# renzibei/flashws

Hardware: AMD Instinct MI355X
Metric: GiB/s masked WS payload unmasked, device-resident frame batch; % HBM roofline (higher is better)
Workload: dtype u8; 1 GPU; C2: device-resident 65536 x 4 KiB masked BIN frames, descriptor-mode unmask of the packed (sorted) batch, one launch (fws_gpu_unmask_sorted); frames_per_gpu=65536, payload_bytes_per_frame=4096, wire_bytes_per_gpu=268959744, rotating_buffers=4, parallelism=batch split x1 (no collective)

## Files before the change

flashws_amd/csrc/fws_abi.hip:

```cpp
#include <stdlib.h>
#include <string.h>

#include "fws_internal.h"

namespace {

template <typename T>
int dev_alloc(T **p, uint64_t count) {
    *p = nullptr;
    if (count == 0) count = 1;
    return fws_hip_status(hipMalloc((void **)p, count * sizeof(T)));
}

template <typename T>
void dev_free(T *&p) {
    if (p) (void)hipFree(p);
    p = nullptr;
}

void free_plan(fws_plan_ws &w) {
    dev_free(w.block_sums);
    dev_free(w.cbase);
    dev_free(w.unit_first);
    dev_free(w.unit_rec);
    dev_free(w.total);
    dev_free(w.status);
    dev_free(w.ticket);
    dev_free(w.mode);
    dev_free(w.tx_seam);
}

}

int fws_ctx_ensure_plan(fws_gpu_ctx *ctx, uint64_t frames, uint64_t units) {
    if (frames <= ctx->cap_frames && units <= ctx->cap_units && ctx->plan.cbase) return 0;
    if (frames < ctx->cap_frames) frames = ctx->cap_frames;
    if (units < ctx->cap_units) units = ctx->cap_units;
    free_plan(ctx->plan);
    int r;
    if ((r = dev_alloc(&ctx->plan.block_sums, frames / 1024 + 2))) return r;
    if ((r = dev_alloc(&ctx->plan.cbase, frames + 2))) return r;
    if ((r = dev_alloc(&ctx->plan.unit_first, units + 2))) return r;
    if ((r = dev_alloc(&ctx->plan.unit_rec, 4 * (units + 2)))) return r;
    if ((r = dev_alloc(&ctx->plan.total, 2))) return r;
    if ((r = dev_alloc(&ctx->plan.status, frames / 8 + 2))) return r;
    if ((r = dev_alloc(&ctx->plan.ticket, 2))) return r;
    if ((r = dev_alloc(&ctx->plan.mode, sizeof(fws_plan_mode) / 8))) return r;
    if ((r = dev_alloc(&ctx->plan.tx_seam, 4 * (2 * frames + 2)))) return r;
    if ((r = fws_hip_status(hipMemset(ctx->plan.status, 0, (frames / 8 + 2) * 8)))) return r;
    if ((r = fws_hip_status(hipMemset(ctx->plan.ticket, 0, 8)))) return r;
    if ((r = fws_hip_status(hipMemset(ctx->plan.mode, 0, sizeof(fws_plan_mode))))) return r;
    ctx->plan.status_cap = frames / 8 + 2;
    ctx->plan.epoch = 0;
    ctx->cap_frames = frames;
    ctx->cap_units = units;
    ctx->plan.unit_cap = units + 1;
    return 0;
}

int fws_ctx_ensure_seam(fws_gpu_ctx *ctx, uint64_t span) {
    const uint64_t words = 2 * (span / 4096 + 2);
    if (words <= ctx->seam_cap) return 0;
    dev_free(ctx->seam);
    ctx->seam_cap = 0;
    if (int r = fws_hip_status(hipMalloc((void **)&ctx->seam, words * 4))) return r;
    ctx->seam_cap = words;
    return 0;
}

int fws_ctx_ensure_msg(fws_gpu_ctx *ctx, uint64_t frames) {
    fws_msg_ws &m = ctx->msg;
    if (!m.cnext) {
        if (int r = dev_alloc(&m.cnext, 1)) return r;
    }
    if (frames <= m.cap && m.descs) return 0;
    if (frames < m.cap) frames = m.cap;
    dev_free(m.descs);
    dev_free(m.ctl_off);
    dev_free(m.agg);
    dev_free(m.pre);
    m.cap = 0;
    int r;
    if ((r = dev_alloc(&m.descs, frames + 1))) return r;
    if ((r = dev_alloc(&m.ctl_off, frames + 1))) return r;
    if ((r = dev_alloc(&m.agg, 8 * (frames / 256 + 2)))) return r;
    if ((r = dev_alloc(&m.pre, 8 * (frames / 256 + 2)))) return r;
    if ((r = fws_hip_status(hipMemset(m.agg, 0, 8 * (frames / 256 + 2) * 8)))) return r;
    if ((r = fws_hip_status(hipMemset(m.pre, 0, 8 * (frames / 256 + 2) * 8)))) return r;
    m.cap = frames;
    m.last_epoch = 0;
    return 0;
}

extern "C" {

__attribute__((visibility("default"))) int fws_internal_decode_counters(fws_gpu_ctx *ctx, uint32_t *out, int n) {
    if (!ctx || !out || n <= 0 || !ctx->dec.counters) return FWS_ERR_INVALID;
    if (n > 64) n = 64;
    return fws_hip_status(hipMemcpy(out, ctx->dec.counters, (size_t)n * 4, hipMemcpyDeviceToHost));
}

__attribute__((visibility("default"))) int fws_internal_plan_mode(fws_gpu_ctx *ctx, uint64_t *out5) {
    if (!ctx || !out5 || !ctx->plan.mode) return FWS_ERR_INVALID;
    return fws_hip_status(hipMemcpy(out5, ctx->plan.mode, 5 * 8, hipMemcpyDeviceToHost));
}

__attribute__((visibility("default"))) int fws_internal_decode_parse(fws_gpu_ctx *ctx, const void *dev_wire,
                                                                     uint64_t len, fws_frame_info *dev_frames,
                                                                     uint32_t cap, fws_decode_result *dev_result,
                                                                     void *stream) {
    if (!ctx || !dev_result || (len && !dev_wire) || (cap && !dev_frames) || ((uintptr_t)dev_wire & 15u))
        return FWS_ERR_INVALID;
    int r;
    if ((r = fws_hip_status(hipSetDevice(ctx->device))) || (r = fws_decode_prepare(ctx, len, cap, false))) return r;
    return fws_launch_decode(ctx, (uint8_t *)const_cast<void *>(dev_wire), len, dev_frames, cap, dev_result, nullptr,
                             (hipStream_t)stream);
}

int fws_gpu_abi_version(void) { return FWS_GPU_ABI_VERSION; }

int fws_gpu_device_count(int *count) {
    if (!count) return FWS_ERR_INVALID;
    *count = 0;
    hipError_t e = hipGetDeviceCount(count);
    if (e == hipErrorNoDevice) { *count = 0; return 0; }
    return fws_hip_status(e);
}

int fws_gpu_ctx_create(int device, fws_gpu_ctx **out) {
    if (!out) return FWS_ERR_INVALID;
    *out = nullptr;
    int n = 0;
    int r = fws_gpu_device_count(&n);
    if (r) return r;
    if (device < 0 || device >= n) return FWS_ERR_NO_DEVICE;
    hipDeviceProp_t prop;
    if ((r = fws_hip_status(hipGetDeviceProperties(&prop, device)))) return r;
// ... 319 lines not shown
```

flashws_amd/csrc/fws_internal.h:

```cpp
#pragma once

#include <hip/hip_runtime.h>
#include <stdint.h>

#include "fws_gpu.h"

static inline int fws_hip_status(hipError_t e) {
    return e == hipSuccess ? 0 : (FWS_ERR_HIP_BASE - (int)e);
}

constexpr uint64_t kSmallMax = 128u << 10;
constexpr uint32_t kSmallFrames = 256;
constexpr int FWS_SMALL_DECLINED = -30;
int fws_resolve_mode();
int fws_launch_decode_small(uint8_t *wire, uint64_t N, fws_frame_info *frames, uint32_t cap,
                            fws_decode_result *res, hipStream_t s);
struct fws_seg_desc {
    uint64_t cont_off;
    uint64_t hs_off;
    uint32_t u;
    uint32_t key;
    uint32_t L;
    uint32_t fcap;
    uint32_t fbase;
// ... 29 lines not shown
static_assert(sizeof(fws_svc_mail) == 128, "one line");
struct alignas(128) fws_svc_dev {
    uint64_t seqn;
    uint32_t quit, ctr, pad[28];
    fws_svc_req req;
};
int fws_launch_rx_service(fws_svc_mail *mail, const fws_svc_mail *poll, fws_svc_dev *dv, uint32_t seq0,
                          uint32_t workers, uint64_t linger_ticks, uint64_t life_ticks, uint32_t trace, hipStream_t s);
int fws_rx_service_trace_read(unsigned long long *out8);
struct fws_rx_service;
fws_rx_service *fws_ctx_rx_service(fws_gpu_ctx *ctx);
void fws_rx_service_destroy(fws_rx_service *v);
int fws_rx_service_run(fws_rx_service *v, uint8_t *base, const fws_seg_desc *descs, const fws_seg_desc *one,
                       uint32_t nseg, fws_frame_info *frames, fws_decode_result *res, uint32_t *flag,
                       uint32_t flag_seq);
int fws_rx_service_post(fws_rx_service *v, uint8_t *base, const fws_seg_desc *descs, uint32_t nseg,
                        fws_frame_info *frames, fws_decode_result *res, uint32_t *flag, uint32_t flag_seq);
int fws_rx_service_wait(fws_rx_service *v, uint32_t *flag, uint32_t flag_seq);
bool fws_rx_service_can_push(const fws_rx_service *v, uint64_t span);
uint32_t fws_rx_service_workers(const fws_rx_service *v);
int fws_rx_service_push(fws_rx_service *v, const uint8_t *src, uint64_t span, uint8_t *out_dev, const fws_seg_desc &d,
                        fws_frame_info *frames, fws_decode_result *res, uint32_t *flag, uint32_t flag_seq);

struct fws_plan_ws {
    uint64_t *block_sums = nullptr;
    uint64_t *cbase = nullptr;
    uint32_t *unit_first = nullptr;
    uint32_t *unit_rec = nullptr;
    uint64_t *total = nullptr;
    uint64_t *status = nullptr;
    uint32_t *ticket = nullptr;
    uint64_t *mode = nullptr;
    uint32_t *tx_seam = nullptr;
    uint64_t status_cap = 0;
    uint32_t epoch = 0;
    uint64_t unit_cap = 0;
};

struct fws_plan_mode {
    uint64_t byte_space;
    uint64_t s0;
    uint64_t first_po;
    uint64_t last_pe;
    uint64_t n_units;
    uint64_t pad[3];
};

struct fws_node_res {
    uint32_t tail;
    uint32_t cnt;
    uint32_t ent;
    uint32_t kind;
};
struct fws_tail_rec {
    uint64_t exit;
    uint32_t id;
    uint32_t w;
    uint32_t wst;
    uint32_t pad;
};

struct fws_st_node {
    uint32_t sid;
    uint16_t nx;
    uint16_t tail;
    uint16_t cnt;
    uint8_t wt;
    uint8_t pad0;
    uint32_t pad1;
};

struct fws_decode_ws {
    uint64_t max_tiles = 0;
    uint64_t max_surv = 0;
    uint32_t *tile_count = nullptr;
    uint32_t *counters = nullptr;
    uint32_t *cnt_base = nullptr;
    uint32_t parity = 0;
// ... 131 lines not shown
```

flashws_amd/csrc/outplan_kernels.hip:

```cpp
#include "fws_device.h"
#include "fws_internal.h"
#include "outplan_common.h"

namespace fwsk {

template <typename Desc, int kF>
__global__ __launch_bounds__(kBlock) void k_out_plan(const Desc *__restrict__ d, uint32_t n, OutPlanArgs a) {
    out_plan_block<Desc, kF>(d, n, a, plan_block_order(a.ticket));
}

}

using namespace fwsk;

int fws_plan_next_epoch(fws_plan_ws &ws, hipStream_t s) {
    if (++ws.epoch > 0xFFFFu) {
        int r = fws_hip_status(hipMemsetAsync(ws.status, 0, ws.status_cap * 8, s));
        if (r) return r;
        ws.epoch = 1;
    }
    return 0;
}

template <typename Desc>
static int launch_out_plan(const Desc *d, uint32_t n, fws_plan_ws &ws, uint64_t out_cap, uint64_t *out_len,
                           hipStream_t s, const uint32_t *deny = nullptr) {
    if (n == 0) return 0;
    const bool small = n <= 16384u;
    const uint32_t nb = small ? (n + 63u) / 64u : (n + kBlock - 1) / kBlock;
    if (nb > ws.status_cap) return FWS_ERR_CAPACITY;
    int r = fws_plan_next_epoch(ws, s);
    if (r) return r;
    OutPlanArgs a{ws.cbase, ws.unit_first, ws.unit_cap, ws.total, out_len, out_cap, deny, ws.status, ws.ticket, ws.epoch};
    if (small)
        hipLaunchKernelGGL((k_out_plan<Desc, 64>), dim3(nb), dim3(kBlock), 0, s, d, n, a);
    else
        hipLaunchKernelGGL((k_out_plan<Desc, kBlock>), dim3(nb), dim3(kBlock), 0, s, d, n, a);
    return fws_hip_status(hipGetLastError());
}

int fws_launch_gather_plan(const fws_frame_desc *d, uint32_t n, fws_plan_ws &ws, hipStream_t s, uint64_t out_cap,
                           const uint32_t *deny) {
    return launch_out_plan(d, n, ws, out_cap, nullptr, s, deny);
}

int fws_launch_tx_plan(const fws_tx_desc *d, uint32_t n, fws_plan_ws &ws, uint64_t out_cap, uint64_t *out_len,
                       hipStream_t s) {
    return launch_out_plan(d, n, ws, out_cap, out_len, s);
}
```

flashws_amd/csrc/plan_common.h:

```cpp
#pragma once
#include "fws_device.h"

namespace fwsk {

constexpr uint64_t kLbValue = (1ull << 45) - 1;
constexpr uint64_t kLbSorted = 1ull << 45;
constexpr uint64_t kLbAgg = 1ull << 46, kLbPrefix = 2ull << 46;

__device__ __forceinline__ uint64_t lb_load(const uint64_t *p) {
    return __hip_atomic_load(p, __ATOMIC_RELAXED, __HIP_MEMORY_SCOPE_AGENT);
}
__device__ __forceinline__ void lb_store(uint64_t *p, uint64_t v) {
    __hip_atomic_store(p, v, __ATOMIC_RELAXED, __HIP_MEMORY_SCOPE_AGENT);
}

__device__ __forceinline__ uint64_t wave_incl_scan64(uint64_t v, int lane) {
#pragma unroll
    for (int o = 1; o < kWave; o <<= 1) {
        const uint64_t t = __shfl_up(v, o, kWave);
        if (lane >= o) v += t;
    }
    return v;
}

__device__ __forceinline__ uint32_t plan_block_order(uint32_t *ticket) {
    __shared__ uint32_t s_blk;
    if (gridDim.x <= 1024u) return blockIdx.x;
    if (threadIdx.x == 0) s_blk = atomicAdd(ticket, 1u);
    __syncthreads();
    const uint32_t blk = s_blk;
    if (blk == gridDim.x - 1 && threadIdx.x == 0) *ticket = 0u;
    return blk;
}

__device__ __forceinline__ uint64_t block_lookback(uint64_t *status, uint32_t blk, uint64_t agg, bool flag,
                                                   uint32_t epoch, bool *all_flag) {
    __shared__ uint32_t s_pstop[kBlock / kWave];
    __shared__ uint64_t s_lsum[kBlock / kWave];
    __shared__ uint32_t s_lbad[kBlock / kWave];
    const int lane = threadIdx.x & (kWave - 1), w = threadIdx.x / kWave;
    const uint64_t tag = (uint64_t)epoch << 48;
    if (threadIdx.x == 0) lb_store(status + blk, tag | (blk == 0 ? kLbPrefix : kLbAgg) | (flag ? kLbSorted : 0) | agg);
    uint64_t excl = 0;
    bool all = flag;
    for (int64_t j = (int64_t)blk - 1; j >= 0; j -= kBlock) {
        const int64_t idx = j - (int64_t)threadIdx.x;
        uint64_t st = tag | kLbPrefix | kLbSorted;
        if (idx >= 0) {
            do {
                st = lb_load(status + idx);
            } while ((st >> 48) != epoch || (st & (3ull << 46)) == 0);
        }
        const uint64_t pm = __ballot((st & (3ull << 46)) == kLbPrefix);
        if (lane == 0) s_pstop[w] = pm ? (uint32_t)(w * kWave + __builtin_ctzll(pm)) : (uint32_t)kBlock;
        __syncthreads();
        uint32_t stop = kBlock;
#pragma unroll
        for (int i = 0; i < kBlock / kWave; ++i) stop = s_pstop[i] < stop ? s_pstop[i] : stop;
        const bool use = threadIdx.x <= stop && idx >= 0;
        uint64_t v = use ? (st & kLbValue) : 0;
        for (int o = 32; o > 0; o >>= 1) v += __shfl_xor(v, o, kWave);
        const uint64_t vb = __ballot(use && !(st & kLbSorted));
        if (lane == 0) {
            s_lsum[w] = v;
            s_lbad[w] = vb != 0;
        }
        __syncthreads();
#pragma unroll
        for (int i = 0; i < kBlock / kWave; ++i) {
            excl += s_lsum[i];
            all = all && !s_lbad[i];
        }
        __syncthreads();
        if (stop < (uint32_t)kBlock) break;
    }
    if (threadIdx.x == 0 && blk != 0)
        lb_store(status + blk, tag | kLbPrefix | (all ? kLbSorted : 0) | ((excl + agg) & kLbValue));
    *all_flag = all;
    return excl;
}

__device__ __forceinline__ uint32_t wave_max(uint32_t v) {
#pragma unroll
    for (int o = 32; o > 0; o >>= 1) {
        const uint32_t t = (uint32_t)__shfl_xor(v, o, kWave);
        v = t > v ? t : v;
    }
    return v;
}

__device__ __forceinline__ uint64_t readlane64(uint64_t v, int k) {
    const uint32_t lo = __builtin_amdgcn_readlane((uint32_t)v, k), hi = __builtin_amdgcn_readlane((uint32_t)(v >> 32), k);
    return ((uint64_t)hi << 32) | lo;
}

constexpr uint32_t kRunInline = 64;

template <typename Get, typename Fn>
__device__ __forceinline__ void wave_for_runs(uint64_t u0, uint32_t len, Get get, Fn fn) {
    if (wave_max(len) <= kRunInline) {
        const auto ctx = get(-1);
        for (uint32_t k = 0; k < len; ++k) fn(ctx, u0 + k);
        return;
    }
    const int lane = threadIdx.x & (kWave - 1);
    for (int L = 0; L < kWave; ++L) {
        const uint32_t n = __builtin_amdgcn_readlane(len, L);
        if (n == 0) continue;
// ... 27 lines not shown
```

flashws_amd/csrc/unmask_kernels.hip:

```cpp
#include "fws_device.h"
#include "fws_internal.h"
#include "plan_common.h"

namespace fwsk {

#ifndef FWS_UNMASK_WT
#define FWS_UNMASK_WT 1
#endif
template <bool kNT, bool kWT = true>
__device__ __forceinline__ void ustore16(uintptr_t a, u32x4 v) {
    if constexpr (kNT && kWT && FWS_UNMASK_WT != 0) gstore16_wt(a, v);
    else gstore16<kNT>(a, v);
}

constexpr int kPlanItems = 1;
constexpr int kPlanTile = kBlock * kPlanItems;

__device__ __forceinline__ uint64_t wave_incl_scan(uint64_t v, int lane) {
#pragma unroll
    for (int o = 1; o < kWave; o <<= 1) {
        uint64_t t = __shfl_up(v, o, kWave);
        if (lane >= o) v += t;
    }
    return v;
// ... 1 lines not shown

__device__ __forceinline__ uint64_t block_excl_scan(uint64_t v, uint64_t *total) {
    __shared__ uint64_t wsum[kBlock / kWave];
    const int lane = threadIdx.x & (kWave - 1), w = threadIdx.x / kWave;
    uint64_t inc = wave_incl_scan(v, lane);
    if (lane == kWave - 1) wsum[w] = inc;
    __syncthreads();
    uint64_t off = 0, tot = 0;
#pragma unroll
    for (int i = 0; i < kBlock / kWave; ++i) {
        uint64_t s = wsum[i];
        off += (i < w) ? s : 0;
        tot += s;
    }
    __syncthreads();
    *total = tot;
    return off + inc - v;
}

__device__ __forceinline__ uint64_t desc_chunks(const uint8_t *base, const fws_frame_desc &d) {
    return chunks_of((uintptr_t)(base + d.payload_off), d.payload_len);
}

struct PlanArgs {
    uint64_t *cbase;
    uint32_t *unit_first;
    u32x4 *unit_rec;
    uint64_t *total;
    uint64_t *status;
    uint32_t *ticket;
    fws_plan_mode *mode;
    uint64_t unit_cap;
    uint32_t epoch;
};

constexpr uint32_t kRecSlow = 1u << 30;

__device__ __forceinline__ uint32_t rec_clip(uint64_t x, uint64_t U0) {
    return x <= U0 ? 0u : (x >= U0 + 4096u ? 4096u : (uint32_t)(x - U0));
}

__device__ __forceinline__ u32x4 unit_record(uint64_t U0, uint64_t E0, uint64_t E1, uint32_t f, uint64_t poA,
                                             uint64_t peA, uint32_t rkA, bool hasB, uint64_t poB, uint64_t peB,
                                             uint32_t rkB, bool hasC, uint64_t poC) {
    if (U0 < E0 || U0 + 4096u > E1 || (hasC && poC < U0 + 4096u)) return u32x4{f, 0u, kRecSlow, 0u};
    const uint32_t a0 = rec_clip(poA, U0), a1 = rec_clip(peA, U0);
    const uint32_t b0 = hasB ? rec_clip(poB, U0) : 0u, b1 = hasB ? rec_clip(peB, U0) : 0u;
    return u32x4{rkA, hasB ? rkB : 0u, a0 | (a1 << 13), b0 | (b1 << 13)};
}


__global__ __launch_bounds__(kBlock) void k_plan(const uint8_t *base, const fws_frame_desc *__restrict__ d,
                                                 uint32_t n, const uint32_t *__restrict__ n_dev, PlanArgs a) {
    __shared__ uint64_t s_wsum[kBlock / kWave];
    __shared__ uint32_t s_wbad[kBlock / kWave];
    if (n_dev && *n_dev < n) n = *n_dev;
    const int lane = threadIdx.x & (kWave - 1), w = threadIdx.x / kWave;
    const uint32_t blk = plan_block_order(a.ticket);
    if (n == 0) {
        if (blk == 0 && threadIdx.x == 0) {
            a.cbase[0] = 0;
            *a.total = 0;
            *a.mode = fws_plan_mode{0, 0, 0, 0, 0, {0, 0, 0}};
        }
        return;
    }
    const uintptr_t b0 = (uintptr_t)base;
    static_assert(kPlanItems == 1, "k_plan: one frame per thread");
    const uint64_t f = uint64_t(blk) * kPlanTile + threadIdx.x;
    const bool has = f < n, hasB = f + 1 < n, hasC = f + 2 < n;
    fws_frame_desc fa{0, 0, 0, 0}, fb{0, 0, 0, 0};
    if (has) fa = d[f];
    if (hasB) fb = d[f + 1];
    const uint64_t poC = hasC ? d[f + 2].payload_off : 0;
    const uint64_t po0 = d[0].payload_off;
    const uint64_t last_pe = d[n - 1].payload_off + d[n - 1].payload_len;
    const uint64_t poA = fa.payload_off, peA = fa.payload_off + fa.payload_len;
    const uint64_t poB = fb.payload_off, peB = fb.payload_off + fb.payload_len;
    const uint64_t s = has ? chunks_of(b0 + poA, fa.payload_len) : 0;
    const bool srt = !hasB || (peA >= poA && peA <= poB);
    const uint64_t inc = wave_incl_scan64(s, lane);
    const uint64_t bad = __ballot(!srt);
    if (lane == kWave - 1) {
        s_wsum[w] = inc;
        s_wbad[w] = bad != 0;
    }
    __syncthreads();
    uint64_t run0 = inc - s, agg = 0;
    bool blk_sorted = true;
#pragma unroll
    for (int i = 0; i < kBlock / kWave; ++i) {
        run0 += i < w ? s_wsum[i] : 0;
        agg += s_wsum[i];
        blk_sorted = blk_sorted && !s_wbad[i];
    }
    bool all_sorted;
    const uint64_t prefix = block_lookback(a.status, blk, agg, blk_sorted, a.epoch, &all_sorted);
    const uint64_t Sa = (b0 + po0) & ~uint64_t(15);
    const uint64_t S = Sa - b0;
    const uint64_t cap = a.unit_cap;
    const uint64_t nus = b0 + last_pe > Sa ? (b0 + last_pe - Sa + 4095u) / 4096u : 0;
    uint64_t run = prefix + run0;
    uint64_t cu = 0, cue = 0, bu = 0, bue = 0;
    if (has) {
        a.cbase[f] = run;
        if (s) {
            cu = (run + kUnitChunks - 1) / kUnitChunks;
            cue = (run + s + kUnitChunks - 1) / kUnitChunks;
        }
        run += s;
        bu = f == 0 ? 0 : (b0 + poA >= Sa ? (b0 + poA - Sa + 4095u) / 4096u : cap);
        bue = !hasB ? nus : (b0 + poB >= Sa ? (b0 + poB - Sa + 4095u) / 4096u : 0);
        if (f == n - 1) {
            a.cbase[n] = run;
            *a.total = run;
            const bool dense = all_sorted && nus + 1 <= cap && (last_pe - S) <= 2u * (run * 16u) + 65536u;
            fws_plan_mode m{dense ? 1ull : 0ull, S, po0, last_pe, nus, {0, 0, 0}};
            *a.mode = m;
        }
    }
    if (cue > cap) cue = cap;
    if (bue > cap) bue = cap;
    if (!all_sorted) bue = bu;
    if (cue < cu) cue = cu;
    if (bue < bu) bue = bu;
    wave_fill_runs(a.unit_first, cu, (uint32_t)(cue - cu), (uint32_t)f, lane);
    struct RecCtx {
        uint64_t poA, peA, poB, peB, poC;
        uint32_t f, rkA, rkB;
        bool hasB, hasC;
    };
    const RecCtx mine{poA, peA, poB, peB, poC, (uint32_t)f, aligned_key(fa.key, fa.phase, b0 + poA),
                      aligned_key(fb.key, fb.phase, b0 + poB), hasB, hasC};
    wave_for_runs(
        bu, (uint32_t)(bue - bu),
        [&](int L) -> RecCtx {
            if (L < 0) return mine;
            return RecCtx{readlane64(mine.poA, L), readlane64(mine.peA, L), readlane64(mine.poB, L),
                          readlane64(mine.peB, L), readlane64(mine.poC, L),
                          (uint32_t)__builtin_amdgcn_readlane(mine.f, L), (uint32_t)__builtin_amdgcn_readlane(mine.rkA, L),
                          (uint32_t)__builtin_amdgcn_readlane(mine.rkB, L),
                          __builtin_amdgcn_readlane((int)mine.hasB, L) != 0,
                          __builtin_amdgcn_readlane((int)mine.hasC, L) != 0};
        },
        [&](const RecCtx &c, uint64_t u) {
            a.unit_rec[u] = unit_record(Sa + 4096u * u, b0 + po0, b0 + last_pe, c.f, b0 + c.poA, b0 + c.peA, c.rkA,
                                        c.hasB, b0 + c.poB, b0 + c.peB, c.rkB, c.hasC, b0 + c.poC);
        });
}

__global__ __launch_bounds__(kBlock) void k_mask_single(uint8_t *base, fws_frame_desc single) {
    const uintptr_t a0 = (uintptr_t)(base + single.payload_off);
    const uintptr_t lo = a0, hi = a0 + single.payload_len;
    const uint64_t total = chunks_of(a0, single.payload_len);
    const uint64_t n_units = (total + kUnitChunks - 1) / kUnitChunks;
    const uint32_t rk = aligned_key(single.key, single.phase, a0);
    const uintptr_t safe = a0 & ~uintptr_t(15);
    const int lane = threadIdx.x & (kWave - 1);
    const uint64_t nwaves = uint64_t(gridDim.x) * (kBlock / kWave);
    for (uint64_t u = uint64_t(blockIdx.x) * (kBlock / kWave) + __builtin_amdgcn_readfirstlane(threadIdx.x / kWave); u < n_units;
         u += nwaves) {
        uintptr_t ca[kUnmaskU];
        bool live[kUnmaskU], full[kUnmaskU];
        u32x4 v[kUnmaskU];
#pragma unroll
        for (int j = 0; j < kUnmaskU; ++j) {
            const uint64_t g = u * kUnitChunks + uint64_t(j) * kWave + lane;
            live[j] = g < total;
            ca[j] = safe + (uintptr_t)(g << 4);
            full[j] = live[j] && ca[j] >= lo && ca[j] + 16u <= hi;
            v[j] = gload16(full[j] ? ca[j] : safe);
        }
#pragma unroll
        for (int j = 0; j < kUnmaskU; ++j) {
            if (full[j]) gstore16(ca[j], v[j] ^ rk);
            else if (live[j]) xor_partial_chunk(ca[j], lo, hi, rk);
        }
    }
}

__device__ __forceinline__ void unmask_one_chunk(uint8_t *base, const fws_frame_desc *__restrict__ d,
// ... 520 lines not shown
        }
        return;
    }
    const fws_frame_desc d0 = d[flo], d1 = d[fhi];
    const uint64_t CB1 = cbase[flo + 1];
    const uintptr_t a0 = (uintptr_t)(base + d0.payload_off), a1 = (uintptr_t)(base + d1.payload_off);
    const uint64_t A0 = (uint64_t)(a0 & ~uintptr_t(15)) - (cbase[flo] << 4);
    const uint64_t A1 = (uint64_t)(a1 & ~uintptr_t(15)) - (CB1 << 4);
    const uint32_t R0 = aligned_key(d0.key, d0.phase, a0), R1 = aligned_key(d1.key, d1.phase, a1);
    const uint64_t S1 = (fhi > flo) ? CB1 : ~0ull;
    uintptr_t ca[J];
    bool live[J], s1[J];
#pragma unroll
    for (int j = 0; j < J; ++j) {
        const uint64_t g = g0 + uint64_t(j) * kWave;
        s1[j] = g >= S1;
        ca[j] = (uintptr_t)((s1[j] ? A1 : A0) + (g << 4));
        live[j] = g < total;
    }
    const uintptr_t safe = a0 & ~uintptr_t(15);
    u32x4 v[J];
#pragma unroll
    for (int j = 0; j < J; ++j) v[j] = gload16<kNT>(live[j] ? ca[j] : safe);
#pragma unroll
    for (int j = 0; j < J; ++j) {
        if (!live[j]) continue;
        const uintptr_t lo = s1[j] ? a1 : a0, hi = s1[j] ? a1 + d1.payload_len : a0 + d0.payload_len;
        const uint32_t rk = s1[j] ? R1 : R0;
        if (ca[j] >= lo && ca[j] + 16u <= hi) ustore16<kNT>(ca[j], v[j] ^ rk);
        else store_partial(ca[j], v[j], rk, lo, hi);
    }
}

template <bool kNT>
__global__ __launch_bounds__(kBlock) __attribute__((amdgpu_waves_per_eu(8))) void k_unmask_desc(uint8_t *base, const fws_frame_desc *__restrict__ d,
                                                        uint32_t n, const uint64_t *__restrict__ cbase,
                                                        const uint32_t *__restrict__ unit_first,
                                                        const u32x4 *__restrict__ unit_rec,
                                                        const uint64_t *__restrict__ total_ptr,
                                                        const fws_plan_mode *__restrict__ mode, uint64_t unit_cap) {
    if (n == 0) return;
    const int lane = threadIdx.x & (kWave - 1);
    const uint64_t nwaves = uint64_t(gridDim.x) * (kBlock / kWave);
    const uint64_t u0 = uint64_t(blockIdx.x) * (kBlock / kWave) + __builtin_amdgcn_readfirstlane(threadIdx.x / kWave);
    const u32x4 rec0 = unit_rec[u0 < unit_cap ? u0 : unit_cap - 1];
    const fws_plan_mode pm = *mode;
    const uint64_t total = *total_ptr;
    if (pm.byte_space) {
        u32x4 rec = rec0;
        for (uint64_t u = u0; u < pm.n_units; u += nwaves) {
            const u32x4 next = (u + nwaves < pm.n_units) ? unit_rec[u + nwaves] : rec;
            byte_space_unit<kNT>(base, d, n, rec, pm, u, lane);
            rec = next;
        }
        return;
    }
    const uint64_t n_units = (total + kUnitChunks - 1) / kUnitChunks;
    for (uint64_t u = u0; u < n_units; u += nwaves)
        chunk_space_unit<kNT>(base, d, n, cbase, unit_first, unit_cap, total, n_units, u, lane);
}

#ifndef FWS_SORTED_WPE
#define FWS_SORTED_WPE 6
#endif
__device__ __forceinline__ uint32_t sorted_owner(const fws_frame_desc *__restrict__ d, uint32_t n, uintptr_t b0,
                                                 uint64_t U0, uint64_t po0, uint64_t u, float rate) {
    if (U0 < po0 || n == 1) return 0u;
    const float gf = (float)(uint32_t)u * rate;
    uint64_t g = (uint32_t)__builtin_amdgcn_readfirstlane((int)(gf < 4.0e9f ? (uint32_t)gf : 0xFFFFFFFFu));
    g = g >= 1u ? g - 1u : 0u;
    if (g > n - 1u) g = n - 1u;
    uint64_t p[4];
#pragma unroll
    for (int k = 0; k < 4; ++k) p[k] = b0 + d[g + k < n ? g + k : n - 1u].payload_off;
#pragma unroll
    for (int k = 0; k < 3; ++k) {
        const uint64_t i = g + k;
        if (i < n && p[k] <= U0 && (i + 1u >= n || p[k + 1] > U0)) return (uint32_t)i;
    }
    uint32_t lo = 0, hi = n;
    while (lo < hi) {
        const uint32_t mid = lo + (hi - lo) / 2u;
        if (b0 + d[mid].payload_off <= U0) lo = mid + 1u;
        else hi = mid;
    }
    return lo - 1u;
}
// ... 505 lines not shown
    return old;
}

static int g_stream_variant = 0;
static int g_stream_utf8_pf = 1;
extern "C" __attribute__((visibility("default"))) int fws_internal_set_stream_utf8_pf(int on) {
    const int old = g_stream_utf8_pf;
    g_stream_utf8_pf = on != 0;
    return old;
}
extern "C" __attribute__((visibility("default"))) int fws_internal_set_stream_variant(int v) {
    const int old = g_stream_variant;
    if (v >= 0 && v <= 3) g_stream_variant = v;
    return old;
}

static int grid_for_units(uint64_t units, int cap = kCapStream) {
    if (g_grid_cap > 0) cap = g_grid_cap;
    uint64_t blocks = (units + (kBlock / kWave) - 1) / (kBlock / kWave);
    if (blocks > (uint64_t)cap) blocks = (uint64_t)cap;
    if (blocks < 1) blocks = 1;
    return (int)blocks;
}

int fws_launch_mask_single(void *dev_ptr, uint64_t n, uint32_t key, uint32_t phase, hipStream_t s) {
    if (n == 0) return 0;
    fws_frame_desc one{0, n, key, phase};
    const uint64_t chunks = ((((uintptr_t)dev_ptr) + n + 15u) >> 4) - (((uintptr_t)dev_ptr) >> 4);
    const uint64_t units = (chunks + kUnitChunks - 1) / kUnitChunks;
    hipLaunchKernelGGL(k_mask_single, dim3(grid_for_units(units)), dim3(kBlock), 0, s, (uint8_t *)dev_ptr, one);
    return fws_hip_status(hipGetLastError());
}

int fws_launch_plan(const uint8_t *base, const fws_frame_desc *d, uint32_t n, const uint32_t *n_dev,
                    fws_plan_ws &ws, hipStream_t s) {
    const uint32_t nb = (n + kPlanTile - 1) / kPlanTile;
    if (nb == 0) return 0;
    if (nb > ws.status_cap) return FWS_ERR_CAPACITY;
    int r = fws_plan_next_epoch(ws, s);
    if (r) return r;
    PlanArgs a{ws.cbase, ws.unit_first, (u32x4 *)ws.unit_rec, ws.total, ws.status, ws.ticket,
               (fws_plan_mode *)ws.mode, ws.unit_cap, ws.epoch};
    hipLaunchKernelGGL(k_plan, dim3(nb), dim3(kBlock), 0, s, base, d, n, n_dev, a);
    return fws_hip_status(hipGetLastError());
}

namespace fwsk {
__global__ __launch_bounds__(kBlock) void k_check_sorted(const fws_frame_desc *__restrict__ d, uint32_t n,
                                                         uint32_t *__restrict__ bad) {
    const uint32_t i = blockIdx.x * kBlock + threadIdx.x;
    bool v = false;
    if (i < n) {
        const uint64_t e = d[i].payload_off + d[i].payload_len;
        v = e < d[i].payload_off || (i + 1 < n && e > d[i + 1].payload_off);
    }
    const uint64_t m = __ballot(v);
    if (m && (threadIdx.x & 63) == (uint32_t)__ffsll((unsigned long long)m) - 1u) atomicMin(bad, i);
}
}

int fws_launch_check_sorted(const fws_frame_desc *d, uint32_t n, uint32_t *bad, hipStream_t s) {
    hipError_t e = hipMemsetAsync(bad, 0xFF, sizeof(uint32_t), s);
    if (e != hipSuccess) return fws_hip_status(e);
    if (n) hipLaunchKernelGGL(fwsk::k_check_sorted, dim3((n + fwsk::kBlock - 1) / fwsk::kBlock), dim3(fwsk::kBlock), 0,
                              s, d, n, bad);
    return fws_hip_status(hipGetLastError());
}

int fws_launch_unmask_sorted(uint8_t *base, const fws_frame_desc *d, uint32_t n, uint64_t max_span,
                             hipStream_t s) {
    if (n == 0) return 0;
    const uint64_t units = max_span / 4096u + 2u;
    if (g_sorted_early == 3)
        hipLaunchKernelGGL((k_unmask_sorted<true, true>), dim3(grid_for_units(units, kCapSorted)), dim3(kBlock), 0, s, base, d, n);
    else if (g_sorted_early)
// ... 37 lines not shown
                               n_dev, unit_first, units, nullptr, nullptr);
        else if (v == 1)
            hipLaunchKernelGGL((k_unmask_stream<true, false, true>), grid, blk, 0, s, (uint8_t *)base, N, frames, cap,
                               n_dev, unit_first, units, nullptr, nullptr);
        else if (v == 2)
            hipLaunchKernelGGL((k_unmask_stream<false, false, false>), grid, blk, 0, s, (uint8_t *)base, N, frames,
                               cap, n_dev, unit_first, units, nullptr, nullptr);
        else
            hipLaunchKernelGGL((k_unmask_stream<false, false, true>), grid, blk, 0, s, (uint8_t *)base, N, frames,
                               cap, n_dev, unit_first, units, nullptr, nullptr);
    } else {
        if (g_stream_utf8_pf && (v == 1 || v == 3))
            hipLaunchKernelGGL((k_unmask_stream<true, true, true, true>), grid, blk, 0, s, (uint8_t *)base, N, frames,
                               cap, n_dev, unit_first, units, utf8_ok, seam);
        else if (g_stream_utf8_pf)
            hipLaunchKernelGGL((k_unmask_stream<true, true, false, true>), grid, blk, 0, s, (uint8_t *)base, N, frames,
                               cap, n_dev, unit_first, units, utf8_ok, seam);
        else if (v == 1 || v == 3)
            hipLaunchKernelGGL((k_unmask_stream<true, true, true>), grid, blk, 0, s, (uint8_t *)base, N, frames, cap,
                               n_dev, unit_first, units, utf8_ok, seam);
        else
            hipLaunchKernelGGL((k_unmask_stream<true, true, false>), grid, blk, 0, s, (uint8_t *)base, N, frames, cap,
                               n_dev, unit_first, units, utf8_ok, seam);
        hipLaunchKernelGGL(k_utf8_seam, dim3((unsigned)((units + kBlock - 1) / kBlock)), dim3(kBlock), 0, s,
                           (const uint8_t *)base, N, frames, cap, n_dev, unit_first, units, utf8_ok, seam);
    }
    return fws_hip_status(hipGetLastError());
}

int fws_launch_unmask(uint8_t *base, const fws_frame_desc *d, uint32_t n, const uint32_t *n_dev,
                      const fws_plan_ws &ws, uint64_t max_chunks, hipStream_t s) {
    const uint64_t units = (max_chunks + kUnitChunks - 1) / kUnitChunks;
    hipLaunchKernelGGL(k_unmask_desc<true>, dim3(grid_for_units(units)), dim3(kBlock), 0, s, base, d, n, ws.cbase,
                       ws.unit_first, (const u32x4 *)ws.unit_rec, ws.total, (const fws_plan_mode *)ws.mode, ws.unit_cap);
    return fws_hip_status(hipGetLastError());
}

static int g_unmask_any = 0;
extern "C" __attribute__((visibility("default"))) int fws_internal_set_unmask_any(int on) {
    const int old = g_unmask_any;
    g_unmask_any = on != 0;
    return old;
}
bool fws_unmask_any_on() { return g_unmask_any != 0; }

int fws_launch_unmask_any(uint8_t *base, const fws_frame_desc *d, uint32_t n, uint64_t *queue, uint32_t qcap,
                          uint32_t *qcnt, uint32_t *qnext, uint32_t piece_grid, hipStream_t s) {
    if (n == 0) return 0;
    uint64_t blocks = (n + (kBlock / kWave) - 1) / (kBlock / kWave);
    if (blocks > (1u << 20)) blocks = 1u << 20;
    hipLaunchKernelGGL(k_unmask_any<true>, dim3((unsigned)blocks), dim3(kBlock), 0, s, base, d, n, queue, qcap, qcnt,
                       qnext);
    hipLaunchKernelGGL(k_unmask_pieces<true>, dim3(piece_grid ? piece_grid : 1u), dim3(kBlock), 0, s, base, d, queue,
                       qcap, qcnt);
    return fws_hip_status(hipGetLastError());
}
```

flashws_amd/gpu.py:

```python
import ctypes as C

import numpy as np
import torch

from . import _lib
from ._lib import (DECODE_JOB, FRAME_DESC, FRAME_INFO, DECODE_RESULT, MSG_CARRY, MSG_INFO, MSG_READ, MSG_RESULT,
                   RX_EVENT, TX_DESC, FwsError, GenParams, check, lib)


def _stream_handle(stream=None):
    s = stream if stream is not None else torch.cuda.current_stream()
    return C.c_void_p(s.cuda_stream)


def _ptr(t):
    return C.c_void_p(t.data_ptr())


_hip = None


def hip_stream():
    global _hip
    if _hip is None:
# ... 579 lines not shown
    def send(self, frames, out_cap=None):
        n = len(frames)
        bufs = [np.frombuffer(bytes(p), dtype=np.uint8).copy() for p, _, _, _ in frames]
        ptrs = np.array([b.ctypes.data if len(b) else 0 for b in bufs], dtype=np.uint64)
        lens = np.array([len(b) for b in bufs], dtype=np.uint64)
        types = np.array([f[1] for f in frames], dtype=np.uint32)
        last = np.array([1 if f[2] else 0 for f in frames], dtype=np.uint8)
        keys = np.array([f[3] & 0xFFFFFFFF for f in frames], dtype=np.uint32)
        cap = int(lens.sum()) + 14 * n if out_cap is None else out_cap
        out = np.zeros(max(cap, 1), dtype=np.uint8)
        ol = C.c_uint64(0)
        rc = lib().fws_tx_session_send(self.h, ptrs.ctypes.data, lens.ctypes.data, types.ctypes.data,
                                       last.ctypes.data, keys.ctypes.data, n, out.ctypes.data, cap, C.byref(ol))
        return rc, out[:ol.value].tobytes() if rc == 0 else b"", ol.value

    def last_msg_not_fin(self):
        v = C.c_uint8(0)
        check("fws_tx_session_state", lib().fws_tx_session_state(self.h, C.byref(v)))
        return v.value

    def close(self):
        if self.h:
            lib().fws_tx_session_destroy(self.h)
            self.h = None

    def __del__(self):
        try:
            self.close()
        except Exception:
            pass


def plan_mode(ctx):
    out = (C.c_uint64 * 5)()
    check("fws_internal_plan_mode", lib().fws_internal_plan_mode(ctx.h, out))
    return dict(zip(("byte_space", "s0", "first_po", "last_pe", "n_units"), list(out)))


def decode_counters(ctx):
    out = (C.c_uint32 * 16)()
    check("fws_internal_decode_counters", lib().fws_internal_decode_counters(ctx.h, out, 16))
    return {"survivors": out[0], "frames": out[3], "failed": out[9] != 0, "big_super_tiles": out[12]}


class RxPipe:

    def __init__(self, device=0, max_batch_bytes=1 << 28, max_frames=1 << 17, depth=3, utf8=False):
        h = C.c_void_p()
        check("fws_rx_pipe_create", lib().fws_rx_pipe_create(device, max_batch_bytes, max_frames, depth,
                                                             1 if utf8 else 0, C.byref(h)))
        self.h = h
        self.max_frames = max_frames
        self.utf8 = utf8

    def submit(self, batch, n=None):
        t = C.c_uint64()
        n = batch.numel() if n is None else n
        check("fws_rx_pipe_submit", lib().fws_rx_pipe_submit(self.h, C.c_void_p(batch.data_ptr()), n, C.byref(t)))
        return t.value

    def wait(self, ticket, copy_frames=True):
        fp, up = C.c_void_p(), C.c_void_p()
        nf = C.c_uint64()
        res = np.zeros(1, dtype=DECODE_RESULT)
        check("fws_rx_pipe_wait", lib().fws_rx_pipe_wait(self.h, ticket, C.byref(fp), C.byref(nf),
                                                         C.c_void_p(res.ctypes.data), C.byref(up)))
        frames = None
        if copy_frames and nf.value:
            raw = (C.c_uint8 * (nf.value * FRAME_INFO.itemsize)).from_address(fp.value)
# ... 37 lines not shown
```

Measured before the change: 3059 GiB/s.

## Add address-space unmask mode for unsorted descriptor batches via per-unit frame tables

Adds a new plan path for descriptor batches that are not sorted by payload offset. The plan kernel builds a per-4KiB-unit address table with linked lists of frames and records the payload extent per block. When the extent is dense enough, the unmask kernel walks units by address instead of falling back to the slow unsorted path. The workload here is a sorted batch, so the plan kernel mostly takes the early-exit branch that only writes a block marker. The cost is extra workspace, extra stores and lookback logic in the plan kernel.

```diff
diff --git a/flashws_amd/csrc/fws_abi.hip b/flashws_amd/csrc/fws_abi.hip
--- a/flashws_amd/csrc/fws_abi.hip
+++ b/flashws_amd/csrc/fws_abi.hip
@@ -28,6 +28,9 @@
     dev_free(w.ticket);
     dev_free(w.mode);
     dev_free(w.tx_seam);
+    dev_free(w.addr_tab);
+    dev_free(w.addr_next);
+    dev_free(w.addr_blk);
 }
 
 }
@@ -47,9 +50,14 @@
     if ((r = dev_alloc(&ctx->plan.ticket, 2))) return r;
     if ((r = dev_alloc(&ctx->plan.mode, sizeof(fws_plan_mode) / 8))) return r;
     if ((r = dev_alloc(&ctx->plan.tx_seam, 4 * (2 * frames + 2)))) return r;
+    if ((r = dev_alloc(&ctx->plan.addr_tab, 2 * (units + 2)))) return r;
+    if ((r = dev_alloc(&ctx->plan.addr_next, frames + 2))) return r;
+    if ((r = dev_alloc(&ctx->plan.addr_blk, 2 * (frames / 8 + 2)))) return r;
     if ((r = fws_hip_status(hipMemset(ctx->plan.status, 0, (frames / 8 + 2) * 8)))) return r;
     if ((r = fws_hip_status(hipMemset(ctx->plan.ticket, 0, 8)))) return r;
     if ((r = fws_hip_status(hipMemset(ctx->plan.mode, 0, sizeof(fws_plan_mode))))) return r;
+    if ((r = fws_hip_status(hipMemset(ctx->plan.addr_tab, 0, 2 * (units + 2) * 8)))) return r;
+    if ((r = fws_hip_status(hipMemset(ctx->plan.addr_blk, 0, 2 * (frames / 8 + 2) * 8)))) return r;
     ctx->plan.status_cap = frames / 8 + 2;
     ctx->plan.epoch = 0;
     ctx->cap_frames = frames;
@@ -103,6 +111,12 @@
 __attribute__((visibility("default"))) int fws_internal_plan_mode(fws_gpu_ctx *ctx, uint64_t *out5) {
     if (!ctx || !out5 || !ctx->plan.mode) return FWS_ERR_INVALID;
     return fws_hip_status(hipMemcpy(out5, ctx->plan.mode, 5 * 8, hipMemcpyDeviceToHost));
+}
+
+__attribute__((visibility("default"))) int fws_internal_plan_mode8(fws_gpu_ctx *ctx, uint64_t *out8) {
+    if (!ctx || !out8 || !ctx->plan.mode) return FWS_ERR_INVALID;
+    static_assert(sizeof(fws_plan_mode) == 8 * 8, "fws_plan_mode: 8 words");
+    return fws_hip_status(hipMemcpy(out8, ctx->plan.mode, sizeof(fws_plan_mode), hipMemcpyDeviceToHost));
 }
 
 __attribute__((visibility("default"))) int fws_internal_decode_parse(fws_gpu_ctx *ctx, const void *dev_wire,
diff --git a/flashws_amd/csrc/fws_internal.h b/flashws_amd/csrc/fws_internal.h
--- a/flashws_amd/csrc/fws_internal.h
+++ b/flashws_amd/csrc/fws_internal.h
@@ -85,6 +85,9 @@
     uint32_t *ticket = nullptr;
     uint64_t *mode = nullptr;
     uint32_t *tx_seam = nullptr;
+    uint64_t *addr_tab = nullptr;
+    uint32_t *addr_next = nullptr;
+    uint64_t *addr_blk = nullptr;
     uint64_t status_cap = 0;
     uint32_t epoch = 0;
     uint64_t unit_cap = 0;
@@ -96,7 +99,9 @@
     uint64_t first_po;
     uint64_t last_pe;
     uint64_t n_units;
-    uint64_t pad[3];
+    uint64_t addr_space;
+    uint64_t min_po;
+    uint64_t max_pe;
 };
 
 struct fws_node_res {
diff --git a/flashws_amd/csrc/outplan_kernels.hip b/flashws_amd/csrc/outplan_kernels.hip
--- a/flashws_amd/csrc/outplan_kernels.hip
+++ b/flashws_amd/csrc/outplan_kernels.hip
@@ -17,6 +17,8 @@
     if (++ws.epoch > 0xFFFFu) {
         int r = fws_hip_status(hipMemsetAsync(ws.status, 0, ws.status_cap * 8, s));
         if (r) return r;
+        if (ws.addr_tab && (r = fws_hip_status(hipMemsetAsync(ws.addr_tab, 0, 2 * ws.unit_cap * 8, s)))) return r;
+        if (ws.addr_blk && (r = fws_hip_status(hipMemsetAsync(ws.addr_blk, 0, 2 * ws.status_cap * 8, s)))) return r;
         ws.epoch = 1;
     }
     return 0;
diff --git a/flashws_amd/csrc/plan_common.h b/flashws_amd/csrc/plan_common.h
--- a/flashws_amd/csrc/plan_common.h
+++ b/flashws_amd/csrc/plan_common.h
@@ -34,7 +34,7 @@
 }
 
 __device__ __forceinline__ uint64_t block_lookback(uint64_t *status, uint32_t blk, uint64_t agg, bool flag,
-                                                   uint32_t epoch, bool *all_flag) {
+                                                   uint32_t epoch, bool *all_flag, bool *prev_flag = nullptr) {
     __shared__ uint32_t s_pstop[kBlock / kWave];
     __shared__ uint64_t s_lsum[kBlock / kWave];
     __shared__ uint32_t s_lbad[kBlock / kWave];
@@ -42,7 +42,7 @@
     const uint64_t tag = (uint64_t)epoch << 48;
     if (threadIdx.x == 0) lb_store(status + blk, tag | (blk == 0 ? kLbPrefix : kLbAgg) | (flag ? kLbSorted : 0) | agg);
     uint64_t excl = 0;
-    bool all = flag;
+    bool all = true;
     for (int64_t j = (int64_t)blk - 1; j >= 0; j -= kBlock) {
         const int64_t idx = j - (int64_t)threadIdx.x;
         uint64_t st = tag | kLbPrefix | kLbSorted;
@@ -74,6 +74,8 @@
         __syncthreads();
         if (stop < (uint32_t)kBlock) break;
     }
+    if (prev_flag) *prev_flag = all;
+    all = all && flag;
     if (threadIdx.x == 0 && blk != 0)
         lb_store(status + blk, tag | kLbPrefix | (all ? kLbSorted : 0) | ((excl + agg) & kLbValue));
     *all_flag = all;
diff --git a/flashws_amd/csrc/unmask_kernels.hip b/flashws_amd/csrc/unmask_kernels.hip
--- a/flashws_amd/csrc/unmask_kernels.hip
+++ b/flashws_amd/csrc/unmask_kernels.hip
@@ -57,7 +57,64 @@
     fws_plan_mode *mode;
     uint64_t unit_cap;
     uint32_t epoch;
+    uint64_t *addr_tab;
+    uint32_t *addr_next;
+    uint64_t *addr_blk;
 };
+
+constexpr uint32_t kAddrNone = 0xFFFFFFFFu;
+__device__ __forceinline__ uint64_t addr_entry(uint32_t epoch, uint32_t f) { return ((uint64_t)epoch << 48) | f; }
+__device__ __forceinline__ bool addr_live(uint64_t e, uint32_t epoch) { return (e >> 48) == epoch; }
+constexpr uint64_t kAddrOff = (1ull << 48) - 1u;
+constexpr uint64_t kAddrPrefixMax = 16384;
+
+struct AddrFrame {
+    uint64_t au, aue;
+    uint64_t lo, hi;
+    uint64_t old;
+    uint32_t f;
+    bool live, listed;
+};
+
+__device__ __forceinline__ AddrFrame addr_frame(uintptr_t b0, uint64_t cap, bool has, uint32_t f,
+                                                const fws_frame_desc &fd) {
+    AddrFrame q{0, 0, kAddrOff, 0, 0, f, false, false};
+    const uint64_t po = fd.payload_off, pe = po + fd.payload_len;
+    q.live = has && fd.payload_len != 0 && pe > po;
+    if (!q.live) return q;
+    const uint64_t Ba = b0 & ~uint64_t(15);
+    const uint64_t rel = b0 + po - Ba, uf = rel >> 12;
+    const bool on_edge = (rel & 4095u) == 0;
+    q.au = on_edge ? uf : uf + 1u;
+    q.aue = ((b0 + pe - 1u - Ba) >> 12) + 1u;
+    if (q.aue > cap) q.aue = cap;
+    if (q.aue < q.au) q.aue = q.au;
+    q.listed = !on_edge && uf < cap;
+    q.old = uf;
+    q.lo = po < kAddrOff ? po : kAddrOff;
+    q.hi = pe < kAddrOff ? pe : kAddrOff;
+    return q;
+}
+
+__device__ __forceinline__ void addr_frame_list(const PlanArgs &a, AddrFrame &q) {
+    if (q.listed)
+        q.old = atomicExch((unsigned long long *)(a.addr_tab + 2u * q.old + 1u),
+                           (unsigned long long)addr_entry(a.epoch, q.f));
+}
+
+__device__ __forceinline__ void addr_frame_finish(const PlanArgs &a, const AddrFrame &q, uint64_t &lo, uint64_t &hi) {
+    const uint32_t ep = a.epoch;
+    uint64_t *const tab = a.addr_tab;
+    const uint32_t f = q.f;
+    wave_for_runs(q.au, (uint32_t)(q.aue - q.au),
+                  [&](int L) { return L < 0 ? f : (uint32_t)__builtin_amdgcn_readlane(f, L); },
+                  [&](uint32_t fl, uint64_t u) { tab[2u * u] = addr_entry(ep, fl); });
+    if (q.listed) a.addr_next[f] = addr_live(q.old, ep) ? (uint32_t)q.old : kAddrNone;
+    if (q.live) {
+        lo = q.lo < lo ? q.lo : lo;
+        hi = q.hi > hi ? q.hi : hi;
+    }
+}
 
 constexpr uint32_t kRecSlow = 1u << 30;
 
@@ -79,6 +136,7 @@
                                                  uint32_t n, const uint32_t *__restrict__ n_dev, PlanArgs a) {
     __shared__ uint64_t s_wsum[kBlock / kWave];
     __shared__ uint32_t s_wbad[kBlock / kWave];
+    __shared__ uint64_t s_wmin[kBlock / kWave], s_wmax[kBlock / kWave], s_total;
     if (n_dev && *n_dev < n) n = *n_dev;
     const int lane = threadIdx.x & (kWave - 1), w = threadIdx.x / kWave;
     const uint32_t blk = plan_block_order(a.ticket);
@@ -86,7 +144,7 @@
         if (blk == 0 && threadIdx.x == 0) {
             a.cbase[0] = 0;
             *a.total = 0;
-            *a.mode = fws_plan_mode{0, 0, 0, 0, 0, {0, 0, 0}};
+            *a.mode = fws_plan_mode{0, 0, 0, 0, 0, 0, 0, 0};
         }
         return;
     }
@@ -119,8 +177,15 @@
         agg += s_wsum[i];
         blk_sorted = blk_sorted && !s_wbad[i];
     }
-    bool all_sorted;
-    const uint64_t prefix = block_lookback(a.status, blk, agg, blk_sorted, a.epoch, &all_sorted);
+    const bool addr = a.addr_tab != nullptr;
+    const bool early = addr && !blk_sorted;
+    AddrFrame mine_a{};
+    if (early) {
+        mine_a = addr_frame(b0, a.unit_cap, has, (uint32_t)f, fa);
+        addr_frame_list(a, mine_a);
+    }
+    bool all_sorted, prev_sorted;
+    const uint64_t prefix = block_lookback(a.status, blk, agg, blk_sorted, a.epoch, &all_sorted, &prev_sorted);
     const uint64_t Sa = (b0 + po0) & ~uint64_t(15);
     const uint64_t S = Sa - b0;
     const uint64_t cap = a.unit_cap;
@@ -140,8 +205,13 @@
             a.cbase[n] = run;
             *a.total = run;
             const bool dense = all_sorted && nus + 1 <= cap && (last_pe - S) <= 2u * (run * 16u) + 65536u;
-            fws_plan_mode m{dense ? 1ull : 0ull, S, po0, last_pe, nus, {0, 0, 0}};
-            *a.mode = m;
+            a.mode->byte_space = dense ? 1ull : 0ull;
+            a.mode->s0 = S;
+            a.mode->first_po = po0;
+            a.mode->last_pe = last_pe;
+            a.mode->n_units = nus;
+            if (!addr || all_sorted) a.mode->addr_space = 0;
+            else s_total = run;
         }
     }
     if (cue > cap) cue = cap;
@@ -172,6 +242,93 @@
             a.unit_rec[u] = unit_record(Sa + 4096u * u, b0 + po0, b0 + last_pe, c.f, b0 + c.poA, b0 + c.peA, c.rkA,
                                         c.hasB, b0 + c.poB, b0 + c.peB, c.rkB, c.hasC, b0 + c.poC);
         });
+    if (!addr) return;
+    uint64_t *const bw = a.addr_blk + 2u * blk;
+    const uint64_t tag = (uint64_t)a.epoch << 48;
+    if (all_sorted) {
+        if (threadIdx.x == 0) {
+            lb_store(bw, tag | kAddrOff);
+            lb_store(bw + 1, tag);
+        }
+        return;
+    }
+    if (!early) {
+        mine_a = addr_frame(b0, cap, has, (uint32_t)f, fa);
+        addr_frame_list(a, mine_a);
+    }
+    uint64_t mn = kAddrOff, mx = 0;
+    addr_frame_finish(a, mine_a, mn, mx);
+    if (prev_sorted && blk != 0) {
+        const uint64_t lim = uint64_t(blk) * kPlanTile;
+        if (lim > kAddrPrefixMax) {
+            mx = kAddrOff;
+        } else {
+            for (uint64_t g0 = 0; g0 < lim; g0 += 4u * kBlock) {
+                AddrFrame q[4];
+#pragma unroll
+                for (int j = 0; j < 4; ++j) {
+                    const uint64_t g = g0 + uint64_t(j) * kBlock + threadIdx.x;
+                    const bool ok = g < lim;
+                    fws_frame_desc fd{0, 0, 0, 0};
+                    if (ok) fd = d[g];
+                    q[j] = addr_frame(b0, cap, ok, (uint32_t)g, fd);
+                    addr_frame_list(a, q[j]);
+                }
+#pragma unroll
+                for (int j = 0; j < 4; ++j) addr_frame_finish(a, q[j], mn, mx);
+            }
+        }
+    }
+    auto block_extent = [&](uint64_t &lo, uint64_t &hi) {
+#pragma unroll
+        for (int o = 32; o > 0; o >>= 1) {
+            const uint64_t tl = __shfl_xor(lo, o, kWave), th = __shfl_xor(hi, o, kWave);
+            lo = tl < lo ? tl : lo;
+            hi = th > hi ? th : hi;
+        }
+        __syncthreads();
+        if (lane == 0) {
+            s_wmin[w] = lo;
+            s_wmax[w] = hi;
+        }
+        __syncthreads();
+#pragma unroll
+        for (int i = 0; i < kBlock / kWave; ++i) {
+            lo = s_wmin[i] < lo ? s_wmin[i] : lo;
+            hi = s_wmax[i] > hi ? s_wmax[i] : hi;
+        }
+    };
+    block_extent(mn, mx);
+    if (threadIdx.x == 0) {
+        lb_store(bw, tag | mn);
+        lb_store(bw + 1, tag | mx);
+    }
+    if ((uint64_t)(n - 1u) / kPlanTile != blk) return;
+    for (uint32_t j0 = 0; j0 < blk; j0 += kBlock) {
+        const uint32_t j = j0 + threadIdx.x;
+        if (j >= blk) continue;
+        uint64_t wl, wh;
+        do {
+            wl = lb_load(a.addr_blk + 2u * j);
+        } while ((wl >> 48) != a.epoch);
+        do {
+            wh = lb_load(a.addr_blk + 2u * j + 1u);
+        } while ((wh >> 48) != a.epoch);
+        wl &= kAddrOff;
+        wh &= kAddrOff;
+        mn = wl < mn ? wl : mn;
+        mx = wh > mx ? wh : mx;
+    }
+    block_extent(mn, mx);
+    if (threadIdx.x != 0) return;
+    bool take = mn < mx && mx != kAddrOff;
+    if (take) {
+        const uint64_t span = mx - mn, hi_units = ((b0 + mx - 1u - (b0 & ~uint64_t(15))) >> 12) + 1u;
+        take = hi_units <= cap && span <= 2u * (s_total * 16u) + 65536u && uint64_t(n) * 4096u <= 2u * span;
+    }
+    a.mode->addr_space = take ? (1ull | ((uint64_t)a.epoch << 32)) : 0ull;
+    a.mode->min_po = mn;
+    a.mode->max_pe = mx;
 }
 
 __global__ __launch_bounds__(kBlock) void k_mask_single(uint8_t *base, fws_frame_desc single) {
@@ -758,13 +915,93 @@
     }
 }
 
+
+__device__ __forceinline__ void or_region_masks(const fws_frame_desc &fd, uintptr_t b0, uint64_t U0, uint32_t o0,
+                                                u32x4 (&m)[kUnmaskU]) {
+    const uint64_t po = b0 + fd.payload_off;
+    const uint32_t l = rec_clip(po, U0), h = rec_clip(po + fd.payload_len, U0);
+    const uint32_t r = aligned_key(fd.key, fd.phase, po);
+    if (h <= l) return;
+#pragma unroll
+    for (int j = 0; j < kUnmaskU; ++j) {
+        const uint32_t o = o0 + (uint32_t)j * 1024u;
+        if (o + 16u <= l || o >= h) continue;
+        m[j] |= u32x4{r & byte_sel32(o, l, h), r & byte_sel32(o + 4u, l, h), r & byte_sel32(o + 8u, l, h),
+                      r & byte_sel32(o + 12u, l, h)};
+    }
+}
+
+__device__ __forceinline__ fws_frame_desc ld_desc(const fws_frame_desc *p) {
+    const uint64_t *q = (const uint64_t *)p;
+    const uint64_t a = q[0], b = q[1], c = q[2];
+    return fws_frame_desc{a, b, (uint32_t)c, (uint32_t)(c >> 32)};
+}
+
+template <bool kNT>
+__device__ __forceinline__ void addr_space_unit(uint8_t *base, const fws_frame_desc *__restrict__ d, uint32_t n,
+                                                const uint64_t *__restrict__ tab, const uint32_t *__restrict__ next,
+                                                uint32_t epoch, uint64_t E0, uint64_t E1, uint64_t U, int lane) {
+    const uintptr_t b0 = (uintptr_t)base;
+    const uint64_t U0 = (b0 & ~uintptr_t(15)) + 4096u * U;
+    const uint64_t ec = tab[2u * U], eh = tab[2u * U + 1u];
+    const bool hasA = addr_live(ec, epoch) && (uint32_t)ec < n, hasH = addr_live(eh, epoch) && (uint32_t)eh < n;
+    if (!hasA && !hasH) return;
+    const uint32_t fA = hasA ? (uint32_t)ec : 0u, fH = hasH ? (uint32_t)eh : 0u;
+    const fws_frame_desc da = ld_desc(d + fA), dh = ld_desc(d + fH);
+    const uint32_t nx = hasH ? next[fH] : kAddrNone;
+    const uint64_t c0 = U0 + uint64_t(lane) * 16u;
+    const bool inner = U0 >= E0 && U0 + 4096u <= E1;
+    u32x4 v[kUnmaskU];
+    if (inner && nx == kAddrNone) {
+        const uint64_t poA = hasA ? b0 + da.payload_off : U0, peA = hasA ? poA + da.payload_len : U0;
+        const uint64_t poB = b0 + dh.payload_off, peB = poB + dh.payload_len;
+        const u32x4 rec = unit_record(U0, E0, E1, fA, poA, peA, hasA ? aligned_key(da.key, da.phase, poA) : 0u, hasH,
+                                      poB, peB, aligned_key(dh.key, dh.phase, poB), false, 0);
+        u32x4 mk[kUnmaskU];
+        fast_unit_masks(rec, lane, mk);
+#pragma unroll
+        for (int j = 0; j < kUnmaskU; ++j) v[j] = gload16<kNT>(c0 + uint64_t(j) * 1024u);
+#pragma unroll
+        for (int j = 0; j < kUnmaskU; ++j)
+            if (mk[j].x | mk[j].y | mk[j].z | mk[j].w) ustore16<kNT>(c0 + uint64_t(j) * 1024u, v[j] ^ mk[j]);
+        return;
+    }
+    u32x4 m[kUnmaskU];
+#pragma unroll
+    for (int j = 0; j < kUnmaskU; ++j) m[j] = u32x4{0u, 0u, 0u, 0u};
+    uint32_t o0 = (uint32_t)lane * 16u;
+    asm volatile("" : "+v"(o0));
+    if (hasA) or_region_masks(da, b0, U0, o0, m);
+    if (hasH) {
+        or_region_masks(dh, b0, U0, o0, m);
+        uint32_t f = nx;
+#pragma unroll 1
+        for (uint32_t k = 1; f < n && f != fH && k < n; ++k) {
+            f = (uint32_t)__builtin_amdgcn_readfirstlane((int)f);
+            const fws_frame_desc fd = ld_desc(d + f);
+            const uint32_t fn = next[f];
+            or_region_masks(fd, b0, U0, o0, m);
+            f = fn;
+        }
+    }
+    const uint64_t safe = (E1 - 1u) & ~uint64_t(15);
+#pragma unroll
+    for (int j = 0; j < kUnmaskU; ++j) {
+        const uint64_t c = c0 + uint64_t(j) * 1024u;
+        v[j] = gload16<kNT>(c < E1 ? c : safe);
+    }
+    slow_unit_store<kNT>(c0, E0, E1, v, m);
+}
+
 template <bool kNT>
 __global__ __launch_bounds__(kBlock) __attribute__((amdgpu_waves_per_eu(8))) void k_unmask_desc(uint8_t *base, const fws_frame_desc *__restrict__ d,
                                                         uint32_t n, const uint64_t *__restrict__ cbase,
                                                         const uint32_t *__restrict__ unit_first,
                                                         const u32x4 *__restrict__ unit_rec,
                                                         const uint64_t *__restrict__ total_ptr,
-                                                        const fws_plan_mode *__restrict__ mode, uint64_t unit_cap) {
+                                                        const fws_plan_mode *__restrict__ mode, uint64_t unit_cap,
+                                                        const uint64_t *__restrict__ addr_tab,
+                                                        const uint32_t *__restrict__ addr_next) {
     if (n == 0) return;
     const int lane = threadIdx.x & (kWave - 1);
     const uint64_t nwaves = uint64_t(gridDim.x) * (kBlock / kWave);
@@ -779,6 +1016,17 @@
             byte_space_unit<kNT>(base, d, n, rec, pm, u, lane);
             rec = next;
         }
+        return;
+    }
+    if (pm.addr_space & 1u) {
+        const uintptr_t b0 = (uintptr_t)base;
+        const uint64_t E0 = b0 + pm.min_po, E1 = b0 + pm.max_pe, Ba = b0 & ~uintptr_t(15);
+        const uint64_t ulo = (E0 - Ba) >> 12;
+        uint64_t uhi = ((E1 - 1u - Ba) >> 12) + 1u;
+        if (uhi > unit_cap) uhi = unit_cap;
+        const uint32_t epoch = (uint32_t)(pm.addr_space >> 32) & 0xFFFFu;
+        for (uint64_t u = ulo + u0; u < uhi; u += nwaves)
+            addr_space_unit<kNT>(base, d, n, addr_tab, addr_next, epoch, E0, E1, u, lane);
         return;
     }
     const uint64_t n_units = (total + kUnitChunks - 1) / kUnitChunks;
@@ -1350,6 +1598,13 @@
     return fws_hip_status(hipGetLastError());
 }
 
+static int g_plan_addr = 1;
+extern "C" __attribute__((visibility("default"))) int fws_internal_set_plan_addr(int on) {
+    const int old = g_plan_addr;
+    g_plan_addr = on != 0;
+    return old;
+}
+
 int fws_launch_plan(const uint8_t *base, const fws_frame_desc *d, uint32_t n, const uint32_t *n_dev,
                     fws_plan_ws &ws, hipStream_t s) {
     const uint32_t nb = (n + kPlanTile - 1) / kPlanTile;
@@ -1357,8 +1612,10 @@
     if (nb > ws.status_cap) return FWS_ERR_CAPACITY;
     int r = fws_plan_next_epoch(ws, s);
     if (r) return r;
+    const bool addr = g_plan_addr && ws.addr_tab && ws.addr_next && ws.addr_blk;
     PlanArgs a{ws.cbase, ws.unit_first, (u32x4 *)ws.unit_rec, ws.total, ws.status, ws.ticket,
-               (fws_plan_mode *)ws.mode, ws.unit_cap, ws.epoch};
+               (fws_plan_mode *)ws.mode, ws.unit_cap, ws.epoch, addr ? ws.addr_tab : nullptr, ws.addr_next,
+               ws.addr_blk};
     hipLaunchKernelGGL(k_plan, dim3(nb), dim3(kBlock), 0, s, base, d, n, n_dev, a);
     return fws_hip_status(hipGetLastError());
 }
@@ -1462,7 +1719,8 @@
                       const fws_plan_ws &ws, uint64_t max_chunks, hipStream_t s) {
     const uint64_t units = (max_chunks + kUnitChunks - 1) / kUnitChunks;
     hipLaunchKernelGGL(k_unmask_desc<true>, dim3(grid_for_units(units)), dim3(kBlock), 0, s, base, d, n, ws.cbase,
-                       ws.unit_first, (const u32x4 *)ws.unit_rec, ws.total, (const fws_plan_mode *)ws.mode, ws.unit_cap);
+                       ws.unit_first, (const u32x4 *)ws.unit_rec, ws.total, (const fws_plan_mode *)ws.mode, ws.unit_cap,
+                       (const uint64_t *)ws.addr_tab, (const uint32_t *)ws.addr_next);
     return fws_hip_status(hipGetLastError());
 }
 
diff --git a/flashws_amd/gpu.py b/flashws_amd/gpu.py
--- a/flashws_amd/gpu.py
+++ b/flashws_amd/gpu.py
@@ -635,9 +635,11 @@
 
 
 def plan_mode(ctx):
-    out = (C.c_uint64 * 5)()
-    check("fws_internal_plan_mode", lib().fws_internal_plan_mode(ctx.h, out))
-    return dict(zip(("byte_space", "s0", "first_po", "last_pe", "n_units"), list(out)))
+    out = (C.c_uint64 * 8)()
+    check("fws_internal_plan_mode8", lib().fws_internal_plan_mode8(ctx.h, out))
+    m = dict(zip(("byte_space", "s0", "first_po", "last_pe", "n_units"), list(out)[:5]))
+    m.update(addr_space=int(out[5]) & 1, min_po=int(out[6]), max_pe=int(out[7]))
+    return m
 
 
 def decode_counters(ctx):
```

Measured after the change: 3059 GiB/s (median of 3 runs). No clear change (+0.0%).
